# Cathoven-AI/Montreal-Forced-Aligner

Hardware: AMD Instinct MI355X
Metric: aligned utterances/sec (whole node), 10 s utts, 5k-state triphone (higher is better)
Workload: dtype f32 scores from 2-way f16-split products (3*2^-22 per term worst case), f64 path costs

## Files before the change

### include/mfa_hip.h

```cpp
#ifndef MFA_HIP_H_
#define MFA_HIP_H_

#include <stddef.h>
#include <stdint.h>

#ifdef __cplusplus
extern "C" {
#endif

#define MFA_API __attribute__((visibility("default")))

typedef struct mfa_ctx mfa_ctx;

MFA_API mfa_ctx *mfa_create(int device_id);
MFA_API void mfa_destroy(mfa_ctx *ctx);
MFA_API const char *mfa_last_error(mfa_ctx *ctx);
MFA_API int mfa_version(void);
MFA_API int mfa_set_stream(mfa_ctx *ctx, void *hip_stream, int use_own);
MFA_API int mfa_synchronize(mfa_ctx *ctx);
MFA_API void *mfa_device_alloc(mfa_ctx *ctx, size_t bytes);
MFA_API int mfa_device_free(mfa_ctx *ctx, void *d_ptr);
MFA_API int mfa_memcpy_h2d(mfa_ctx *ctx, void *d_dst, const void *h_src, size_t bytes);
MFA_API int mfa_memcpy_d2h(mfa_ctx *ctx, void *h_dst, const void *d_src, size_t bytes);
MFA_API int mfa_timer_begin(mfa_ctx *ctx);
MFA_API int mfa_timer_end_ms(mfa_ctx *ctx, float *h_ms);
MFA_API int mfa_kernel_timing(mfa_ctx *ctx, int enable);
MFA_API int mfa_kernel_time_ms(mfa_ctx *ctx, int which, float *h_ms, int *h_launches);
MFA_API int mfa_kernel_time_reset(mfa_ctx *ctx);

typedef struct {
  float sample_frequency;
  float frame_length_ms;
  float frame_shift_ms;
  float preemphasis;
  float low_frequency;
  float high_frequency;
  float cepstral_lifter;
  float energy_floor;
  int32_t num_mel_bins;
  int32_t num_coefficients;
  int32_t snip_edges;
  int32_t remove_dc_offset;
  int32_t use_energy;
  int32_t raw_energy;
} mfa_mfcc_opts;

MFA_API int mfa_mfcc_configure(mfa_ctx *ctx, const mfa_mfcc_opts *opts);
MFA_API int32_t mfa_mfcc_num_frames(mfa_ctx *ctx, int64_t num_samples);
MFA_API int mfa_mfcc_batch(mfa_ctx *ctx, const int16_t *d_pcm, const int64_t *d_sample_off, const int64_t *d_frame_off,
                           int32_t n_utt, int32_t max_frames, float *d_mfcc);

MFA_API int mfa_gather_pcm(int32_t n_utt, const int16_t *const *h_src, const int64_t *h_sample_off, int16_t *h_dst,
                           int32_t n_threads);

MFA_API int64_t mfa_resample_num_samples(int32_t in_hz, int32_t out_hz, int64_t n);
MFA_API int mfa_resample_plan(int32_t in_hz, int32_t out_hz, int32_t *phases, int32_t *in_per_unit, int32_t *max_taps,
                              int32_t *h_first, int32_t *h_taps, float *h_weights);
MFA_API int mfa_resample_plan_general(int32_t in_hz, int32_t out_hz, double cutoff_hz, int32_t zeros, int32_t *phases,
                                      int32_t *in_per_unit, int32_t *max_taps, int32_t *h_first, int32_t *h_taps,
                                      float *h_weights);
MFA_API int32_t mfa_resample_block_outputs(void);
MFA_API int mfa_resample_batch(mfa_ctx *ctx, int32_t in_hz, int32_t out_hz, const int16_t *d_in, const int64_t *d_in_off,
                               int16_t *d_out, const int64_t *d_out_off, const int32_t *d_utt, int32_t n_sel, int64_t max_out);

typedef struct {
  float sample_frequency;
  float frame_length_ms;
  float frame_shift_ms;
  float min_f0;
  float max_f0;
  float soft_min_f0;
  float penalty_factor;
  float lowpass_cutoff;
  float resample_frequency;
  float delta_pitch;
  float nccf_ballast;
  float preemphasis;
  float pov_scale;
  float pov_offset;
  float pitch_scale;
  int32_t lowpass_filter_width;
  int32_t upsample_filter_width;
  int32_t snip_edges;
// ... 208 lines not shown
```

### montreal_forced_aligner_amd/_lib.py

```python
from __future__ import annotations

import ctypes as C
import os
import subprocess
from pathlib import Path

_PKG = Path(__file__).resolve().parent
_SO = Path(os.environ["MFA_HIP_SO"]).resolve() if os.environ.get("MFA_HIP_SO") else _PKG / "libmfa_hip.so"
_SOURCES = ["api.hip", "mfcc.hip", "feats.hip", "gmm.hip", "gmm_band.hip", "gmm_pack.cpp", "score_plan.cpp", "viterbi.hip", "viterbi_general.hip",
            "fmllr.hip", "gmm_acc.hip", "gmm_acc_host.cpp", "resample.hip", "resample_plan.cpp", "pitch.hip", "pitch_plan.cpp", "compress.hip", "align_equal.hip", "align_equal_host.cpp",
            "lda_acc.hip", "lda_acc_host.cpp", "mllt_acc.hip", "mllt_acc_host.cpp", "tree_acc.hip", "tree_acc_host.cpp"]
_LIB = None


class MfaHipError(RuntimeError):
    pass


STATUS_REASONS = {
    2: "no alignment within the retry beam",
    3: "token capacity exceeded (device decoder status 3)",
    4: "back-pointer capacity exceeded (device decoder status 4)",
    5: "unsupported graph: a state with more than 64 arcs of a kind (device decoder status 5)",
    6: "internal consistency check failed (device decoder status 6)",
# ... 69 lines not shown
               "resample_plan.hpp", "pitch_plan.hpp", "compress_math.hpp", "gmm_acc_math.hpp", "tid_lookup.hpp", "align_equal_math.hpp", "lda_acc_math.hpp", "mllt_acc_math.hpp", "tree_acc_math.hpp")
    deps = srcs + [src_dir / h for h in headers] + [_PKG.parent / "include" / "mfa_hip.h"]
    if not force and _SO.exists() and all(_SO.stat().st_mtime >= d.stat().st_mtime for d in deps if d.exists()):
        return _SO
    hipcc = os.environ.get("HIPCC", "/opt/rocm/bin/hipcc")
    cmd = [hipcc, "--offload-arch=gfx950", "-O3", "-ffp-contract=off", "-fPIC", "-shared", "-std=c++17",
           "-fvisibility=hidden"] + os.environ.get("MFA_HIPCC_FLAGS", "").split() + ["-o", str(_SO)] + [str(s) for s in srcs]
    if verbose:
        print(" ".join(cmd))
    subprocess.check_call(cmd)
    return _SO


_vp, _i32, _i64, _f32 = C.c_void_p, C.c_int32, C.c_int64, C.c_float
SIGNATURES = {
    "mfa_create": (_vp, [C.c_int]),
    "mfa_destroy": (None, [_vp]),
    "mfa_last_error": (C.c_char_p, [_vp]),
    "mfa_version": (C.c_int, []),
    "mfa_set_stream": (C.c_int, [_vp, _vp, C.c_int]),
    "mfa_synchronize": (C.c_int, [_vp]),
    "mfa_device_alloc": (_vp, [_vp, C.c_size_t]),
    "mfa_device_free": (C.c_int, [_vp, _vp]),
    "mfa_memcpy_h2d": (C.c_int, [_vp, _vp, _vp, C.c_size_t]),
    "mfa_memcpy_d2h": (C.c_int, [_vp, _vp, _vp, C.c_size_t]),
    "mfa_timer_begin": (C.c_int, [_vp]),
    "mfa_timer_end_ms": (C.c_int, [_vp, C.POINTER(C.c_float)]),
    "mfa_kernel_timing": (C.c_int, [_vp, C.c_int]),
    "mfa_kernel_time_ms": (C.c_int, [_vp, C.c_int, C.POINTER(C.c_float), C.POINTER(C.c_int)]),
    "mfa_kernel_time_reset": (C.c_int, [_vp]),
    "mfa_mfcc_configure": (C.c_int, [_vp, C.POINTER(MfccOpts)]),
    "mfa_mfcc_num_frames": (_i32, [_vp, _i64]),
    "mfa_mfcc_batch": (C.c_int, [_vp, _vp, _vp, _vp, _i32, _i32, _vp]),
    "mfa_gather_pcm": (C.c_int, [_i32, _vp, _vp, _vp, _i32]),
    "mfa_resample_num_samples": (_i64, [_i32, _i32, _i64]),
    "mfa_resample_plan": (C.c_int, [_i32, _i32, _vp, _vp, _vp, _vp, _vp, _vp]),
    "mfa_resample_plan_general": (C.c_int, [_i32, _i32, C.c_double, _i32, _vp, _vp, _vp, _vp, _vp, _vp]),
    "mfa_resample_block_outputs": (_i32, []),
    "mfa_resample_batch": (C.c_int, [_vp, _i32, _i32, _vp, _vp, _vp, _vp, _vp, _i32, _i64]),
    "mfa_pitch_configure": (C.c_int, [_vp, C.POINTER(PitchOpts)]),
    "mfa_pitch_num_frames": (_i32, [_vp, _i64]),
    "mfa_pitch_num_states": (_i32, [_vp]),
    "mfa_pitch_num_columns": (_i32, [_vp]),
    "mfa_pitch_workspace_bytes": (C.c_size_t, [_vp, _i32, _i64, _i64, _i64, _i32]),
    "mfa_pitch_batch": (C.c_int, [_vp, _vp, _vp, _vp, _vp, _vp, _i32, _i32, _vp]),
    "mfa_pitch_process_batch": (C.c_int, [_vp, _vp, _vp, _i32, _i32, _vp, _i32, _i32]),
    "mfa_debug_pitch_stages": (C.c_int, [_vp, C.POINTER(PitchOpts), _vp, _vp, _vp, _vp, _vp, _vp, _vp, _vp, _vp, _vp, _vp, _vp,
                                         _i32, _i32, _vp, _vp, _vp, _vp, _vp, _vp]),
    "mfa_cmvn_stats": (C.c_int, [_vp, _vp, _vp, _i32, _i32, _vp, _vp, _i32, _vp]),
    "mfa_feats_batch": (C.c_int, [_vp, _vp, _vp, _i32, _i32, _i32, _vp, _vp, _i32, _i32, _vp, _i32, _i32, _vp, _vp]),
    "mfa_compress_resident_values": (_i32, []),
    "mfa_compress_batch": (C.c_int, [_vp, _vp, _vp, _i32, _i32, _i32, _i32, _vp, _vp, _i32, _vp, _vp, _vp, _vp]),
    "mfa_debug_compress_host": (C.c_int, [_vp, _i32, _i32, _vp, _vp, _vp, _vp]),
    "mfa_load_gmm": (C.c_int, [_vp, _i32, _i32, _vp, _vp, _vp, _vp]),
    "mfa_gmm_slot": (_i32, [_vp, _i32]),
    "mfa_gmm_sort_pdf_list": (C.c_int, [_vp, _vp, _i32, _vp]),
    "mfa_gmm_sort_pdf_list_keyed": (C.c_int, [_vp, _vp, _vp, _i32, _vp]),
    "mfa_fst_first_frames": (C.c_int, [_i32, _vp, _vp, _i32, _vp]),
    "mfa_debug_gmm_trace": (C.c_int, [_vp, _vp]),
    "mfa_debug_gmm_pack": (C.c_int, [_i32, _i32, _vp, _vp, _vp, _vp, _vp, _vp, _vp, _vp, _vp, _vp, _vp, _vp, _vp, _vp, _vp,
                                      _vp, _vp, _i32, _vp]),
    "mfa_debug_viterbi_stamps": (C.c_int, [_vp, _vp]),
    "mfa_gmm_score_batch": (C.c_int, [_vp, _vp, _vp, _i32, _i32, _vp, _vp, _vp, _vp, _vp, _vp]),
    "mfa_align_batch": (C.c_int, [_vp, C.POINTER(GraphBatch), _vp, _vp, _vp, _vp, _i64, _i64, _i32, _i32, C.POINTER(AlignOpts),
                                  _vp, _vp, _vp, _vp, _vp, _vp]),
    "mfa_align_general_batch": (C.c_int, [_vp, C.POINTER(GraphBatch), _vp, _vp, _vp, _vp, _vp, _i32, _i32, C.POINTER(AlignOpts),
# ... 6 lines not shown
    "mfa_build_score_plans_batch": (C.c_int, [_i32, _vp, _vp, _vp, _vp, _vp, _vp, _i32, _vp, _i32, _i32, _i32, _vp, _vp, _vp, _vp,
                                              _vp, _vp, _vp, _vp, _vp]),
    "mfa_fmllr_acc_batch": (C.c_int, [_vp, _vp, _vp, _i32, _i64, _vp, _vp, _vp, _vp, _i32, _vp, _vp, _vp]),
    "mfa_fmllr_acc_ali_batch": (C.c_int, [_vp, _vp, _vp, _i32, _i64, _vp, _vp, _vp, _i32, _vp, _vp, _vp, _vp, _i32, _vp, _vp, _vp]),
    "mfa_fmllr_stats_model": (C.c_int, [_vp, _i32, _i32, _vp, _vp, _vp]),
    "mfa_gmm_acc_chunk_frames": (_i32, []),
    "mfa_gmm_acc_max_dim": (_i32, []),
    "mfa_gmm_acc_batch": (C.c_int, [_vp, _vp, _i64, _vp, _vp, _vp, _i32, _vp, _vp, _vp, _vp, _vp]),
    "mfa_debug_gmm_acc_host": (C.c_int, [_i32, _i32, _vp, _vp, _vp, _vp, _vp, _i64, _vp, _vp, _vp, _i32, _vp, _vp, _vp, _vp, _vp,
                                          _vp, _i32]),
    "mfa_align_equal_batch": (C.c_int, [_vp, C.POINTER(GraphBatch), _vp, _i64, _i64, _vp, C.c_uint32, _vp, _vp]),
    "mfa_debug_align_equal_host": (C.c_int, [_i32, _vp, _vp, _vp, _vp, _vp, _vp, _vp, _vp, _vp, C.c_uint32, _vp, _vp]),
    "mfa_lda_acc_slab_frames": (_i32, []),
    "mfa_lda_acc_chunk_frames": (_i32, []),
    "mfa_lda_acc_max_dim": (_i32, []),
    "mfa_lda_acc_batch": (C.c_int, [_vp, _vp, _vp, _i32, _i64, _i32, _vp, _vp, _i32, _vp, _vp, _vp, _i32, _i32, _f32, _vp, C.c_uint32,
                                    _vp, _vp, _vp, _vp]),
    "mfa_debug_lda_acc_host": (C.c_int, [_vp, _vp, _i32, _i32, _vp, _vp, _i32, _vp, _vp, _vp, _i32, _i32, _f32, _vp, C.c_uint32,
                                         _vp, _vp, _vp, _vp]),
    "mfa_mllt_acc_chunk_frames": (_i32, []),
    "mfa_mllt_acc_max_dim": (_i32, []),
    "mfa_mllt_acc_batch": (C.c_int, [_vp, _vp, _i64, _vp, _vp, _vp, _i32, _vp, _vp, _vp, _vp]),
    "mfa_debug_mllt_acc_host": (C.c_int, [_i32, _i32, _vp, _vp, _vp, _vp, _vp, _vp, _i64, _vp, _vp, _vp, _vp, _vp, _vp, _i32]),
    "mfa_tree_acc_chunk_frames": (_i32, []),
    "mfa_tree_acc_max_dim": (_i32, []),
    "mfa_tree_acc_batch": (C.c_int, [_vp, _vp, _vp, _i32, _i64, _i32, _vp, _vp, _vp, _vp, _i32, _vp, _i32, _i64, _vp, _vp, _vp, _vp,
                                     _vp, _vp, _vp]),
    "mfa_debug_tree_acc_host": (C.c_int, [_vp, _vp, _i32, _i32, _vp, _vp, _vp, _vp, _i32, _vp, _i32, _i64, _vp, _vp, _vp, _vp, _vp,
                                          _vp, _vp]),
    "mfa_align_workspace_bytes": (C.c_size_t, [_vp, _i32, _i64, C.POINTER(AlignOpts)]),
}


def lib() -> C.CDLL:
    global _LIB
    if _LIB is None:
        if not _SO.exists():
            raise MfaHipError(
                f"{_SO} is missing: build it with `python -c 'import __graft_entry__ as g; g.build()'` "
                "(the alignment path has no CPU fallback)"
            )
        import torch

        try:
            handle = C.CDLL(str(_SO))
        except OSError as e:
            raise MfaHipError(f"cannot load {_SO}: {e}") from e
        for name, (res, args) in SIGNATURES.items():
            fn = getattr(handle, name)
            fn.restype = res
            fn.argtypes = args
        _LIB = handle
    return _LIB


def check(ctx, rc: int, what: str) -> None:
    if rc != 0:
        msg = lib().mfa_last_error(ctx)
        raise MfaHipError(f"{what}: {msg.decode() if msg else 'error'}")


def _ptr(t):
    return None if t is None else C.c_void_p(t.data_ptr())
```

### montreal_forced_aligner_amd/csrc/mfcc.hip

```cpp
#include <algorithm>
#include <cmath>
#include <vector>

#include "ctx.hpp"

namespace {

typedef float v2f __attribute__((ext_vector_type(2)));

constexpr int kNfft = 512;
constexpr int kHalf = 256;
#ifndef MFA_MFCC_WAVES
#define MFA_MFCC_WAVES 8
#endif
constexpr int kWavesPerBlock = MFA_MFCC_WAVES;
constexpr int kFramesPerWave = 16;
constexpr int kFramesPerBlock = kWavesPerBlock * kFramesPerWave;
constexpr int kMaxBins = 32;
constexpr int kMaxCeps = 16;
constexpr int kMaxDct = 384;
constexpr int kMaxPieces = 96;
constexpr int kPieceTaps = 8;
constexpr int kMaxMelW = kMaxPieces * kPieceTaps;
constexpr int kRowPad = 17;
constexpr int kTileFloats = 4 * 16 * kRowPad * 2;
constexpr int kPStride = 273;
constexpr int kPartStride = kMaxPieces + 8;
constexpr int kMelStride = kMaxBins + 8;
constexpr int kPartOff = 4 * kPStride;
constexpr int kMelOff = kPartOff + 4 * kPartStride;
static_assert(kMelOff + 4 * kMelStride <= kTileFloats, "tile reuse");

struct MfccParams {
  int win, shift, nbins, nceps, snip_edges, remove_dc;
  int n_pieces, n_rounds, np_max;
  int raw_energy;
  float log_energy_floor;
  float preemph;
  const float *window;
  const float *tw256;
  const float *tw512;
  const float *melw;
  const int32_t *melinfo;
  const float *dct;
  const float *lifter;
};

#define WAVE_SYNC()                                              \
  do {                                                           \
    __builtin_amdgcn_fence(__ATOMIC_RELEASE, "wavefront");       \
    __builtin_amdgcn_wave_barrier();                             \
    __builtin_amdgcn_fence(__ATOMIC_ACQUIRE, "wavefront");       \
  } while (0)

template <int CTRL>
__device__ __forceinline__ float dpp_f32(float old, float v) {
  return __int_as_float(__builtin_amdgcn_update_dpp(__float_as_int(old), __float_as_int(v), CTRL, 0xF, 0xF, false));
}
template <int CTRL>
__device__ __forceinline__ float dpp_perm(float v) {
  return __int_as_float(__builtin_amdgcn_mov_dpp(__float_as_int(v), CTRL, 0xF, 0xF, true));
}
__device__ __forceinline__ float row_sum_exact(float v) {
  v += dpp_f32<0xB1>(0.0f, v);
// ... 14 lines not shown
template <bool kZero3 = false>
__device__ __forceinline__ void dft4(v2f &a0, v2f &a1, v2f &a2, v2f &a3) {
  const v2f s02 = a0 + a2, d02 = a0 - a2;
  const v2f s13 = kZero3 ? a1 : a1 + a3, d13 = kZero3 ? a1 : a1 - a3;
  a0 = s02 + s13; a2 = s02 - s13;
  a1 = (v2f){d02.x + d13.y, d02.y - d13.x};
  a3 = (v2f){d02.x - d13.y, d02.y + d13.x};
}
template <int kLive = 16>
__device__ __forceinline__ void dft16(v2f (&a)[16]) {
  constexpr float c1 = 0.92387953251128674f, s1 = 0.38268343236508977f, h = 0.70710678118654752f;
#pragma unroll
  for (int na = 0; na < 4; na++) {
    if (na + 12 >= kLive && na + 8 < kLive) dft4<true>(a[na], a[na + 4], a[na + 8], a[na + 12]);
    else dft4<false>(a[na], a[na + 4], a[na + 8], a[na + 12]);
  }
  a[1 + 4] = cmul(a[1 + 4], (v2f){c1, -s1});
  a[1 + 8] = cmul(a[1 + 8], (v2f){h, -h});
  a[1 + 12] = cmul(a[1 + 12], (v2f){s1, -c1});
  a[2 + 4] = cmul(a[2 + 4], (v2f){h, -h});
  a[2 + 8] = (v2f){a[2 + 8].y, -a[2 + 8].x};
  a[2 + 12] = cmul(a[2 + 12], (v2f){-h, -h});
  a[3 + 4] = cmul(a[3 + 4], (v2f){s1, -c1});
  a[3 + 8] = cmul(a[3 + 8], (v2f){-h, -h});
  a[3 + 12] = cmul(a[3 + 12], (v2f){-c1, s1});
#pragma unroll
  for (int kb = 0; kb < 4; kb++) dft4(a[4 * kb], a[4 * kb + 1], a[4 * kb + 2], a[4 * kb + 3]);
#pragma unroll
  for (int kb = 0; kb < 4; kb++)
#pragma unroll
    for (int ka = kb + 1; ka < 4; ka++) { const v2f t = a[4 * kb + ka]; a[4 * kb + ka] = a[4 * ka + kb]; a[4 * ka + kb] = t; }
}

template <int kJ, bool kEnergy = false>
__global__ __launch_bounds__(64 * kWavesPerBlock, 4) void mfcc_kernel(MfccParams p, const int16_t *__restrict__ pcm,
                                                                        const int64_t *__restrict__ sample_off,
                                                                        const int64_t *__restrict__ frame_off,
                                                                        float *__restrict__ out) {
  __shared__ float s_tile[kWavesPerBlock][kTileFloats];
  __shared__ v2f s_tw256[256];
  __shared__ v2f s_tw512[256];
  __shared__ float s_melw[kMaxMelW];
  __shared__ float s_dct[kMaxDct];
  __shared__ v2f s_wnd[256];
  __shared__ int s_info[kMaxPieces + kMaxBins];
  const int utt = blockIdx.y;
  const int lane = threadIdx.x & 63, wave = __builtin_amdgcn_readfirstlane(threadIdx.x >> 6);
  const int q = lane >> 4, i = lane & 15;
  const int64_t s0 = sample_off[utt], n = sample_off[utt + 1] - s0;
  const int64_t f0 = frame_off[utt];
  const int T = (int)(frame_off[utt + 1] - f0);
  if ((int)blockIdx.x * kFramesPerBlock >= T) return;
  for (int k = threadIdx.x; k < 256; k += 64 * kWavesPerBlock) {
    s_tw256[k] = (v2f){p.tw256[2 * k], p.tw256[2 * k + 1]};
    s_tw512[k] = (v2f){p.tw512[2 * k], p.tw512[2 * k + 1]};
    s_wnd[k] = (v2f){p.window[2 * k], p.window[2 * k + 1]};
  }
  for (int k = threadIdx.x; k < p.n_pieces * kPieceTaps; k += 64 * kWavesPerBlock) s_melw[k] = p.melw[k];
  for (int k = threadIdx.x; k < p.nceps * p.nbins; k += 64 * kWavesPerBlock) s_dct[k] = p.dct[k];
  for (int k = threadIdx.x; k < kMaxPieces + kMaxBins; k += 64 * kWavesPerBlock) s_info[k] = p.melinfo[k];
  float *tile = s_tile[wave];
  for (int k = lane; k < kTileFloats; k += 64) tile[k] = 0.0f;
  __syncthreads();
  const int fbase = blockIdx.x * kFramesPerBlock + wave * kFramesPerWave;
  const int nfr = min(kFramesPerWave, T - fbase);
  if (nfr <= 0) return;
  const int16_t *x = pcm + s0;

  const float lift_k = i < p.nceps ? p.lifter[i] : 0.0f;
  v2f *tq = (v2f *)tile + q * (16 * kRowPad);
  float *pq = tile + q * kPStride;
  float *partq = tile + kPartOff + q * kPartStride;
  float *melq = tile + kMelOff + q * kMelStride;

  auto load_frame = [&](int f, unsigned (&raw)[kJ]) {
    const int64_t start = p.snip_edges ? (int64_t)f * p.shift : (int64_t)p.shift * f + p.shift / 2 - p.win / 2;
    const bool fast = start >= 0 && start + 32 * kJ <= n && (((s0 + start) & 1) == 0);
    if (__all(fast)) {
      const unsigned *xs = reinterpret_cast<const unsigned *>(x + start);
#pragma unroll
      for (int j = 0; j < kJ; j++) raw[j] = xs[16 * j + i];
      return;
    }
#pragma unroll
    for (int j = 0; j < kJ; j++) {
      unsigned both = 0;
#pragma unroll
      for (int e = 0; e < 2; e++) {
        const int s = 2 * (16 * j + i) + e;
        unsigned val = 0;
        if (s < p.win) {
          int64_t si = start + s;
          while (si < 0 || si >= n) si = (si < 0) ? (-si - 1) : (2 * n - 1 - si);
          val = (unsigned short)x[si];
        }
        both |= val << (16 * e);
      }
      raw[j] = both;
    }
  };
  auto frame_of = [&](int it) { return fbase + min(4 * it + q, nfr - 1); };

  unsigned nxt[kJ];
  load_frame(frame_of(0), nxt);
  const int npass = (nfr + 3) >> 2;
  for (int it = 0; it < npass; it++) {
    const int f = frame_of(it);
    const bool live = 4 * it + q < nfr;
    int ti = i;
    asm volatile("" : "+v"(ti));
    const v2f *wnd = s_wnd + ti, *tw256 = s_tw256 + ti, *tw512 = s_tw512 + ti;
    v2f a[16];
#pragma unroll
    for (int j = 0; j < 16; j++) a[j] = (v2f){0.0f, 0.0f};
#pragma unroll
    for (int j = 0; j < kJ; j++) a[j] = (v2f){(float)(short)(nxt[j] & 0xFFFFu), (float)(short)(nxt[j] >> 16)};
    if (it + 1 < npass) load_frame(frame_of(it + 1), nxt);
    const bool ok_e = 2 * (16 * (kJ - 1) + i) < p.win, ok_o = 2 * (16 * (kJ - 1) + i) + 1 < p.win;
    auto clear_tail = [&]() {
      if (p.win < 32 * (kJ - 1)) {
#pragma unroll
        for (int j = 8; j < kJ - 1; j++) {
          if (2 * (16 * j + i) >= p.win) a[j].x = 0.0f;
          if (2 * (16 * j + i) + 1 >= p.win) a[j].y = 0.0f;
        }
      }
      if (!ok_e) a[kJ - 1].x = 0.0f;
      if (!ok_o) a[kJ - 1].y = 0.0f;
    };
    clear_tail();
    float sum = 0.0f;
#pragma unroll
    for (int j = 0; j < kJ; j++) sum += a[j].x + a[j].y;
    sum = row_sum_exact(sum);
    const float off = p.remove_dc ? (-sum / (float)p.win) : 0.0f;
#pragma unroll
    for (int j = 0; j < kJ; j++) a[j] += splat(off);
    clear_tail();
    float log_energy = 0.0f;
    auto frame_log_energy = [&]() {
      float e = 0.0f;
#pragma unroll
      for (int j = 0; j < kJ; j++) e = fmaf(a[j].y, a[j].y, fmaf(a[j].x, a[j].x, e));
      e = row_sum_exact(e);
      return __builtin_amdgcn_logf(fmaxf(e, 1.1920928955078125e-07f)) * 0.693147180559945309f;
    };
    if constexpr (kEnergy) { if (p.raw_energy) log_energy = frame_log_energy(); }
    {
      float prev_e[kJ];
#pragma unroll
      for (int j = 0; j < kJ; j++) {
        const float up = a[j > 0 ? j - 1 : 0].y;
        const float carry = j == 0 ? a[0].x : dpp_perm<0x121>(up);
        prev_e[j] = dpp_f32<0x111>(carry, a[j].y);
      }
#pragma unroll
      for (int j = 0; j < kJ; j++) {
        const v2f prev = (v2f){prev_e[j], a[j].x};
        a[j] = (a[j] - splat(p.preemph) * prev) * wnd[16 * j];
      }
    }
    if constexpr (kEnergy) { if (!p.raw_energy) log_energy = frame_log_energy(); }
    dft16<kJ>(a);
#pragma unroll
    for (int k1 = 1; k1 < 16; k1++) a[k1] = cmul(a[k1], tw256[16 * k1]);
#pragma unroll
    for (int k1 = 0; k1 < 16; k1++) tq[k1 * kRowPad + i] = a[k1];
    WAVE_SYNC();
#pragma unroll
    for (int n2 = 0; n2 < 16; n2++) a[n2] = tq[i * kRowPad + n2];
    WAVE_SYNC();
    dft16(a);
#pragma unroll
    for (int k2 = 0; k2 < 16; k2++) {
      const v2f zk = a[k2], own = a[(16 - k2) & 15], far = a[15 - k2];
      const float cx = dpp_f32<0x111>(own.x, dpp_perm<0x140>(far.x));
      const float cy = dpp_f32<0x111>(own.y, dpp_perm<0x140>(far.y));
      float ex = zk.x + cx, ey = zk.y - cy, dx = zk.x - cx, dy = zk.y + cy;
      asm("" : "+v"(ex), "+v"(dx));
      const v2f xk = (v2f){ex, ey} + cmul(tw512[16 * k2], (v2f){dx, dy});
      float pw = 0.25f * fmaf(xk.y, xk.y, xk.x * xk.x);
      if (k2 == 0 && i == 0) pw = 0.25f * (xk.x * xk.x);
      pq[16 * k2 + i] = pw;
    }
    WAVE_SYNC();
    for (int r = 0; r < p.n_rounds; r++) {
      const int piece = 16 * r + i;
      const int pc = min(piece, p.n_pieces - 1);
      const float *wv = s_melw + pc * kPieceTaps;
      const float *pv = pq + s_info[pc];
      float acc = 0.0f;
#pragma unroll
      for (int t = 0; t < kPieceTaps; t++) acc = fmaf(wv[t], pv[t], acc);
      if (piece < p.n_pieces) partq[piece] = acc;
    }
    WAVE_SYNC();
#pragma unroll
    for (int half = 0; half < 2; half++) {
      const int b = i + 16 * half;
      if (b < p.nbins) {
        const int info = s_info[kMaxPieces + b];
        const int first = info & 0xFF, np = info >> 8;
        float e = partq[first];
        for (int r = 1; r < p.np_max; r++) if (r < np) e += partq[first + r];
        melq[b] = __builtin_amdgcn_logf(fmaxf(e, 1.1920928955078125e-07f)) * 0.693147180559945309f;
      }
    }
    WAVE_SYNC();
    if (i < p.nceps) {
      const float *d = s_dct + i * p.nbins;
      float acc = 0.0f;
      for (int b = 0; b < p.nbins; b++) acc = fmaf(d[b], melq[b], acc);
      float c_out = acc * lift_k;
      if constexpr (kEnergy) { if (i == 0) c_out = fmaxf(log_energy, p.log_energy_floor); }
      if (live) out[(f0 + f) * p.nceps + i] = c_out;
    }
    WAVE_SYNC();
  }
}

float mel_scale(float f) { return 1127.0f * logf(1.0f + f / 700.0f); }

}

extern "C" {

MFA_API int mfa_mfcc_configure(mfa_ctx *c, const mfa_mfcc_opts *o) {
  MFA_HIP_CHECK(c, hipSetDevice(c->device));
  int win = (int)(o->sample_frequency * 0.001f * o->frame_length_ms);
  int shift = (int)(o->sample_frequency * 0.001f * o->frame_shift_ms);
  int nfft = 1;
  while (nfft < win) nfft <<= 1;
  if (nfft != kNfft) return c->fail("MFCC kernel supports a 512-point FFT (window %d samples → %d)", win, nfft);
  if (o->num_mel_bins > kMaxBins || o->num_coefficients > kMaxCeps || o->num_coefficients > o->num_mel_bins ||
      o->num_mel_bins * o->num_coefficients > kMaxDct)
    return c->fail("unsupported num_mel_bins/num_coefficients %d/%d", o->num_mel_bins, o->num_coefficients);
  int nb = o->num_mel_bins, nc = o->num_coefficients;
  std::vector<float> window(win);
  double a = 2.0 * M_PI / (win - 1);
  for (int i = 0; i < win; i++) window[i] = (float)pow(0.5 - 0.5 * cos(a * (double)i), 0.85);
  std::vector<float> wpairs(16 * 16 * 2, 0.0f);
  for (int j = 0; j < 16; j++)
    for (int i = 0; i < 16; i++)
      for (int e = 0; e < 2; e++) {
        const int sidx = 2 * (16 * j + i) + e;
        wpairs[2 * (16 * j + i) + e] = sidx < win ? window[sidx] : 0.0f;
      }
  std::vector<float> tw(2 * 256 * 2);
  for (int k = 0; k < 16; k++)
    for (int i = 0; i < 16; i++) {
      const double a256 = 2.0 * M_PI * (double)(i * k) / 256.0, a512 = 2.0 * M_PI * (double)(i + 16 * k) / 512.0;
      tw[2 * (16 * k + i)] = (float)cos(a256);
      tw[2 * (16 * k + i) + 1] = (float)(-sin(a256));
      tw[512 + 2 * (16 * k + i)] = (float)(-sin(a512));
// ... 44 lines not shown
      for (int t = 0; t < best_taps; t++) {
        const int at = q * best_taps + t;
        piecew.push_back(at < len_of[b] ? melw[woff_of[b] + at] : 0.0f);
      }
    }
  }
  std::vector<float> dct((size_t)nc * nb), lifter(nc);
  float norm0 = std::sqrt(1.0f / (float)nb), norm = std::sqrt(2.0f / (float)nb);
  for (int k = 0; k < nc; k++)
    for (int n = 0; n < nb; n++)
      dct[(size_t)k * nb + n] = (k == 0) ? norm0 : (float)(norm * std::cos((double)M_PI / nb * (n + 0.5) * k));
  for (int i = 0; i < nc; i++)
    lifter[i] = o->cepstral_lifter != 0.0f ? (float)(1.0 + 0.5 * o->cepstral_lifter * sin(M_PI * i / o->cepstral_lifter)) : 1.0f;

  return dev_upload_commit<MfaHipDev>(
      c, "the MFCC tables",
      {{&c->d_window, wpairs.data(), wpairs.size() * 4}, {&c->d_twiddle, tw.data(), tw.size() * 4},
       {&c->d_melw, piecew.data(), piecew.size() * 4}, {&c->d_melidx, melinfo.data(), melinfo.size() * 4},
       {&c->d_dct, dct.data(), dct.size() * 4}, {&c->d_lifter, lifter.data(), lifter.size() * 4}},
      [&] {
        c->n_melw = n_pieces; c->mel_np_max = np_max;
        c->mfcc = *o;
        c->win = win; c->shift = shift; c->nfft = nfft;
        c->mfcc_ready = true;
      });
}

MFA_API int32_t mfa_mfcc_num_frames(mfa_ctx *c, int64_t n) {
  if (!c->mfcc_ready) return -1;
  if (c->mfcc.snip_edges) return n < c->win ? 0 : (int32_t)(1 + (n - c->win) / c->shift);
  return (int32_t)((n + c->shift / 2) / c->shift);
}

MFA_API int mfa_mfcc_batch(mfa_ctx *c, const int16_t *d_pcm, const int64_t *d_sample_off, const int64_t *d_frame_off,
                           int32_t n_utt, int32_t max_frames, float *d_mfcc) {
  if (!c->mfcc_ready) return c->fail("mfa_mfcc_configure has not been called");
  if (n_utt <= 0 || max_frames <= 0) return 0;
  if (n_utt > 65535) return c->fail("at most 65535 utterances per MFCC launch (got %d)", n_utt);
  MfccParams p;
  p.win = c->win; p.shift = c->shift; p.nbins = c->mfcc.num_mel_bins; p.nceps = c->mfcc.num_coefficients;
  p.snip_edges = c->mfcc.snip_edges; p.remove_dc = c->mfcc.remove_dc_offset; p.preemph = c->mfcc.preemphasis;
  p.raw_energy = c->mfcc.raw_energy;
  p.log_energy_floor = c->mfcc.energy_floor > 0.0f ? logf(c->mfcc.energy_floor) : -INFINITY;
  p.window = c->d_window.ptr<float>(); p.tw256 = c->d_twiddle.ptr<float>(); p.tw512 = p.tw256 + 512;
  p.melw = c->d_melw.ptr<float>(); p.melinfo = c->d_melidx.ptr<int32_t>(); p.dct = c->d_dct.ptr<float>(); p.lifter = c->d_lifter.ptr<float>();
  p.n_pieces = c->n_melw; p.n_rounds = (c->n_melw + 15) / 16; p.np_max = c->mel_np_max;
  dim3 grid((max_frames + kFramesPerBlock - 1) / kFramesPerBlock, n_utt);
  KernelTimer kt(c, MFA_K_MFCC);
  const bool energy = c->mfcc.use_energy != 0;
  if (c->win <= 32 * 13) {
    if (energy) hipLaunchKernelGGL((mfcc_kernel<13, true>), grid, dim3(64 * kWavesPerBlock), 0, c->stream, p, d_pcm, d_sample_off, d_frame_off, d_mfcc);
    else hipLaunchKernelGGL((mfcc_kernel<13, false>), grid, dim3(64 * kWavesPerBlock), 0, c->stream, p, d_pcm, d_sample_off, d_frame_off, d_mfcc);
  } else {
    if (energy) hipLaunchKernelGGL((mfcc_kernel<16, true>), grid, dim3(64 * kWavesPerBlock), 0, c->stream, p, d_pcm, d_sample_off, d_frame_off, d_mfcc);
    else hipLaunchKernelGGL((mfcc_kernel<16, false>), grid, dim3(64 * kWavesPerBlock), 0, c->stream, p, d_pcm, d_sample_off, d_frame_off, d_mfcc);
  }
  MFA_HIP_CHECK(c, hipGetLastError());
  return 0;
}

}
```

### montreal_forced_aligner_amd/engine.py

```python
from __future__ import annotations

import ctypes as C
from functools import partialmethod
from typing import Dict, List, Optional, Sequence

import numpy as np
import torch

from . import _lib, hostcpu
from ._lib import AlignOpts, GraphBatch, MfccOpts, ScorePlan, _ptr, check
from .frontend import DEFAULT_PITCH, _PITCH_ALIAS, FrontEndStages
from .kaldi_io import Fst
from .model import DiagGmmModel, TransitionModel
from .packing import GraphPacking, PackedGraphs
from .pipeline import Pipeline
from .ragged import _rows_by_group, _speaker_groups, max_len, offsets
from .staging import StagingPool, StagingRing
from .stats import (GmmStats, LdaStats, MlltStats, TreeStats, check_delta_fmllr, fmllr_statistics, gmm_statistics, gmm_statistics_host,
                    lda_statistics, lda_statistics_host, mllt_statistics, mllt_statistics_host, model_arrays, tid_tables, tree_statistics, tree_statistics_host)

STATUS_OK, STATUS_RETRIED, STATUS_FAILED, STATUS_TOKEN_OVERFLOW, STATUS_BP_OVERFLOW, STATUS_UNSUPPORTED = 0, 1, 2, 3, 4, 5

DEFAULT_MFCC = dict(sample_frequency=16000.0, frame_length_ms=25.0, frame_shift_ms=10.0, preemphasis=0.97,
                    low_frequency=20.0, high_frequency=7800.0, cepstral_lifter=22.0, energy_floor=0.0,
# ... 24 lines not shown
        self.use_torch_stream()
        self.mfcc_opts: Optional[MfccOpts] = None
        self.num_ceps = 13
        self.gmm: Optional[DiagGmmModel] = None
        self.slot_class: Optional[np.ndarray] = None
        self._staging = StagingRing(self.device, 3)
        self._pcm_staging = StagingRing(self.device, 2)
        self._nf_checked: Optional[tuple] = None
        self._slab, self._slab_off = None, 0

    def next_staging(self) -> StagingPool:
        return self._staging.next()

    def close(self) -> None:
        if self.ctx:
            self.lib.mfa_destroy(self.ctx)
            self.ctx = None

    def __del__(self):
        try:
            self.close()
        except Exception:
            pass

    def use_torch_stream(self) -> None:
        self.stream = torch.cuda.current_stream(self.device)
        check(self.ctx, self.lib.mfa_set_stream(self.ctx, C.c_void_p(self.stream.cuda_stream), 0), "mfa_set_stream")

    def configure_mfcc(self, **kw) -> None:
        opts = _lib.options(MfccOpts, DEFAULT_MFCC, kw, "MFCC")
        check(self.ctx, self.lib.mfa_mfcc_configure(self.ctx, C.byref(opts)), "mfa_mfcc_configure")
        self.mfcc_opts = opts
        self.num_ceps = int(opts.num_coefficients)

    def load_gmm(self, gmm: DiagGmmModel) -> None:
        po, gc, mi, iv = model_arrays(gmm)
        check(self.ctx, self.lib.mfa_load_gmm(self.ctx, gmm.dim, gmm.num_pdfs, po.ctypes.data, gc.ctypes.data,
                                              mi.ctypes.data, iv.ctypes.data), "mfa_load_gmm")
        self.gmm = gmm
        slots = np.array([self.lib.mfa_gmm_slot(self.ctx, p) for p in range(gmm.num_pdfs)], dtype=np.int32)
        n_gauss = np.diff(gmm.pdf_offsets)
        cls = np.full(gmm.num_pdfs, 5, dtype=np.int32)
        for i, s in enumerate((32, 16, 8, 4, 1)):
            cls[slots == s] = i + 1
        cls[(slots == 32) & (n_gauss <= 32)] = 0
        self.slot_class = cls

    def num_frames(self, num_samples: int) -> int:
        return int(self.lib.mfa_mfcc_num_frames(self.ctx, num_samples))

    def num_frames_array(self, num_samples: np.ndarray) -> np.ndarray:
        n = np.asarray(num_samples, dtype=np.int64)
        if self.mfcc_opts is None:
            self.configure_mfcc()
        o = self.mfcc_opts
        f32 = np.float32
        win = int(f32(f32(o.sample_frequency) * f32(0.001)) * f32(o.frame_length_ms))
        shift = int(f32(f32(o.sample_frequency) * f32(0.001)) * f32(o.frame_shift_ms))
        snip = int(o.snip_edges)
        out = np.where(n < win, 0, 1 + (n - win) // shift) if snip else (n + shift // 2) // shift
        key = (win, shift, snip)
        if self._nf_checked != key:
            for probe in (0, 1, win - 1, win, win + shift - 1, win + shift, 159999, 160000, 160001, 1 << 20):
                ref = (0 if probe < win else 1 + (probe - win) // shift) if snip else (probe + shift // 2) // shift
                if self.num_frames(probe) != ref:
                    raise _lib.MfaHipError("num_frames_array disagrees with mfa_mfcc_num_frames")
# ... 252 lines not shown
```

Before: 264,100.

## Add specialised MFCC kernel path with lane-strided constant tables and fixed mel loops

Adds a specialised MFCC kernel variant that is picked when every mel bin spans at most 8 pieces. It re-lays the twiddle, window, mel-weight and DCT tables in shared memory with a per-lane stride so each lane can read them as 16-byte vectors. The mel-piece and bin loops become fixed-count unrolled loops with per-lane offsets held in registers. The aim is to cut LDS traffic, bank conflicts and loop overhead in the front end, at the cost of higher register pressure and more template instantiations. MFCC is a small share of the whole alignment pipeline, so end-to-end gains are likely small.

```diff
diff --git a/include/mfa_hip.h b/include/mfa_hip.h
--- a/include/mfa_hip.h
+++ b/include/mfa_hip.h
@@ -49,6 +49,7 @@
 MFA_API int32_t mfa_mfcc_num_frames(mfa_ctx *ctx, int64_t num_samples);
 MFA_API int mfa_mfcc_batch(mfa_ctx *ctx, const int16_t *d_pcm, const int64_t *d_sample_off, const int64_t *d_frame_off,
                            int32_t n_utt, int32_t max_frames, float *d_mfcc);
+MFA_API int mfa_mfcc_path(mfa_ctx *ctx);
 
 MFA_API int mfa_gather_pcm(int32_t n_utt, const int16_t *const *h_src, const int64_t *h_sample_off, int16_t *h_dst,
                            int32_t n_threads);
diff --git a/montreal_forced_aligner_amd/_lib.py b/montreal_forced_aligner_amd/_lib.py
--- a/montreal_forced_aligner_amd/_lib.py
+++ b/montreal_forced_aligner_amd/_lib.py
@@ -125,6 +125,7 @@
     "mfa_mfcc_configure": (C.c_int, [_vp, C.POINTER(MfccOpts)]),
     "mfa_mfcc_num_frames": (_i32, [_vp, _i64]),
     "mfa_mfcc_batch": (C.c_int, [_vp, _vp, _vp, _vp, _i32, _i32, _vp]),
+    "mfa_mfcc_path": (C.c_int, [_vp]),
     "mfa_gather_pcm": (C.c_int, [_i32, _vp, _vp, _vp, _i32]),
     "mfa_resample_num_samples": (_i64, [_i32, _i32, _i64]),
     "mfa_resample_plan": (C.c_int, [_i32, _i32, _vp, _vp, _vp, _vp, _vp, _vp]),
@@ -197,6 +198,9 @@
 }
 
 
+_NEWER = {"mfa_mfcc_path"}
+
+
 def lib() -> C.CDLL:
     global _LIB
     if _LIB is None:
@@ -212,6 +216,8 @@
         except OSError as e:
             raise MfaHipError(f"cannot load {_SO}: {e}") from e
         for name, (res, args) in SIGNATURES.items():
+            if name in _NEWER and os.environ.get("MFA_HIP_SO") and not hasattr(handle, name):
+                continue
             fn = getattr(handle, name)
             fn.restype = res
             fn.argtypes = args
diff --git a/montreal_forced_aligner_amd/csrc/mfcc.hip b/montreal_forced_aligner_amd/csrc/mfcc.hip
--- a/montreal_forced_aligner_amd/csrc/mfcc.hip
+++ b/montreal_forced_aligner_amd/csrc/mfcc.hip
@@ -7,6 +7,7 @@
 namespace {
 
 typedef float v2f __attribute__((ext_vector_type(2)));
+typedef float v4f __attribute__((ext_vector_type(4)));
 
 constexpr int kNfft = 512;
 constexpr int kHalf = 256;
@@ -30,6 +31,17 @@
 constexpr int kPartOff = 4 * kPStride;
 constexpr int kMelOff = kPartOff + 4 * kPartStride;
 static_assert(kMelOff + 4 * kMelStride <= kTileFloats, "tile reuse");
+constexpr int kFastRounds = kMaxPieces / 16;
+constexpr int kFastNp = 8;
+static_assert(kMaxPieces + kFastNp <= kPartStride + 1, "a bin's batch of piece sums stays inside its row");
+static_assert(kMelOff % 4 == 0 && kMelStride % 4 == 0 && kTileFloats % 4 == 0, "16-byte reads of the log energies");
+constexpr int kLaneStride = 36;
+constexpr int kGenTw256 = 0, kGenTw512 = 512, kGenWnd = 1024, kGenMelw = 1536, kGenDct = kGenMelw + kMaxMelW,
+              kGenInfo = kGenDct + kMaxDct, kGenConst = kGenInfo + kMaxPieces + kMaxBins;
+constexpr int kFastTab = 16 * kLaneStride;
+constexpr int kFastTw256 = 0, kFastTw512 = kFastTab, kFastWnd = 2 * kFastTab, kFastMelw = 3 * kFastTab,
+              kFastDct = kFastMelw + kMaxMelW, kFastConst = kFastDct + kMaxCeps * kLaneStride;
+static_assert(kMaxBins <= kLaneStride - 4 && kFastMelw % 4 == 0 && kFastDct % 4 == 0, "16-byte units");
 
 struct MfccParams {
   int win, shift, nbins, nceps, snip_edges, remove_dc;
@@ -110,18 +122,15 @@
     for (int ka = kb + 1; ka < 4; ka++) { const v2f t = a[4 * kb + ka]; a[4 * kb + ka] = a[4 * ka + kb]; a[4 * ka + kb] = t; }
 }
 
-template <int kJ, bool kEnergy = false>
+template <int kJ, bool kEnergy, bool kFast>
 __global__ __launch_bounds__(64 * kWavesPerBlock, 4) void mfcc_kernel(MfccParams p, const int16_t *__restrict__ pcm,
                                                                         const int64_t *__restrict__ sample_off,
                                                                         const int64_t *__restrict__ frame_off,
                                                                         float *__restrict__ out) {
-  __shared__ float s_tile[kWavesPerBlock][kTileFloats];
-  __shared__ v2f s_tw256[256];
-  __shared__ v2f s_tw512[256];
-  __shared__ float s_melw[kMaxMelW];
-  __shared__ float s_dct[kMaxDct];
-  __shared__ v2f s_wnd[256];
-  __shared__ int s_info[kMaxPieces + kMaxBins];
+  __shared__ __attribute__((aligned(16))) float s_tile[kWavesPerBlock][kTileFloats];
+  __shared__ __attribute__((aligned(16))) float s_const[kFast ? kFastConst : kGenConst];
+  constexpr int kTw256 = kFast ? kFastTw256 : kGenTw256, kTw512 = kFast ? kFastTw512 : kGenTw512,
+                kWnd = kFast ? kFastWnd : kGenWnd, kMelw = kFast ? kFastMelw : kGenMelw, kDct = kFast ? kFastDct : kGenDct;
   const int utt = blockIdx.y;
   const int lane = threadIdx.x & 63, wave = __builtin_amdgcn_readfirstlane(threadIdx.x >> 6);
   const int q = lane >> 4, i = lane & 15;
@@ -130,13 +139,25 @@
   const int T = (int)(frame_off[utt + 1] - f0);
   if ((int)blockIdx.x * kFramesPerBlock >= T) return;
   for (int k = threadIdx.x; k < 256; k += 64 * kWavesPerBlock) {
-    s_tw256[k] = (v2f){p.tw256[2 * k], p.tw256[2 * k + 1]};
-    s_tw512[k] = (v2f){p.tw512[2 * k], p.tw512[2 * k + 1]};
-    s_wnd[k] = (v2f){p.window[2 * k], p.window[2 * k + 1]};
-  }
-  for (int k = threadIdx.x; k < p.n_pieces * kPieceTaps; k += 64 * kWavesPerBlock) s_melw[k] = p.melw[k];
-  for (int k = threadIdx.x; k < p.nceps * p.nbins; k += 64 * kWavesPerBlock) s_dct[k] = p.dct[k];
-  for (int k = threadIdx.x; k < kMaxPieces + kMaxBins; k += 64 * kWavesPerBlock) s_info[k] = p.melinfo[k];
+    const int at = kFast ? (k & 15) * kLaneStride + 2 * (k >> 4) : 2 * k;
+    s_const[kTw256 + at] = p.tw256[2 * k]; s_const[kTw256 + at + 1] = p.tw256[2 * k + 1];
+    s_const[kTw512 + at] = p.tw512[2 * k]; s_const[kTw512 + at + 1] = p.tw512[2 * k + 1];
+    s_const[kWnd + at] = p.window[2 * k]; s_const[kWnd + at + 1] = p.window[2 * k + 1];
+  }
+  if constexpr (kFast) {
+    for (int k = threadIdx.x; k < kMaxMelW; k += 64 * kWavesPerBlock) {
+      const int piece = k / kPieceTaps, t = k % kPieceTaps;
+      s_const[kMelw + (((piece >> 4) * 2 + (t >> 2)) * 16 + (piece & 15)) * 4 + (t & 3)] = piece < p.n_pieces ? p.melw[k] : 0.0f;
+    }
+    for (int k = threadIdx.x; k < kMaxCeps * kLaneStride; k += 64 * kWavesPerBlock) {
+      const int row = k / kLaneStride, b = k % kLaneStride;
+      s_const[kDct + k] = row < p.nceps && b < p.nbins ? p.dct[row * p.nbins + b] : 0.0f;
+    }
+  } else {
+    for (int k = threadIdx.x; k < p.n_pieces * kPieceTaps; k += 64 * kWavesPerBlock) s_const[kMelw + k] = p.melw[k];
+    for (int k = threadIdx.x; k < p.nceps * p.nbins; k += 64 * kWavesPerBlock) s_const[kDct + k] = p.dct[k];
+    for (int k = threadIdx.x; k < kMaxPieces + kMaxBins; k += 64 * kWavesPerBlock) s_const[kGenInfo + k] = __int_as_float(p.melinfo[k]);
+  }
   float *tile = s_tile[wave];
   for (int k = lane; k < kTileFloats; k += 64) tile[k] = 0.0f;
   __syncthreads();
@@ -145,22 +166,34 @@
   if (nfr <= 0) return;
   const int16_t *x = pcm + s0;
 
-  const float lift_k = i < p.nceps ? p.lifter[i] : 0.0f;
+  auto lane_lifter = [&](int l) { return l < p.nceps ? p.lifter[l] : 0.0f; };
   v2f *tq = (v2f *)tile + q * (16 * kRowPad);
   float *pq = tile + q * kPStride;
   float *partq = tile + kPartOff + q * kPartStride;
   float *melq = tile + kMelOff + q * kMelStride;
-
-  auto load_frame = [&](int f, unsigned (&raw)[kJ]) {
+  auto lane_plan = [&](int l, int (&poff)[kFastRounds], int (&binfo)[2]) {
+#pragma unroll
+    for (int r = 0; r < kFastRounds; r++) poff[r] = p.melinfo[16 * r + l];
+    binfo[0] = p.melinfo[kMaxPieces + l]; binfo[1] = p.melinfo[kMaxPieces + 16 + l];
+  };
+  constexpr bool kKeep = kJ <= 13;
+  float lift_k = 0.0f;
+  int poff[kFastRounds] = {}, binfo[2] = {};
+  if constexpr (kKeep) {
+    lift_k = lane_lifter(i);
+    if constexpr (kFast) lane_plan(i, poff, binfo);
+  }
+
+  auto load_frame = [&](int f, int li, unsigned (&raw)[kJ]) {
     const int64_t start = p.snip_edges ? (int64_t)f * p.shift : (int64_t)p.shift * f + p.shift / 2 - p.win / 2;
     const bool fast = start >= 0 && start + 32 * kJ <= n && (((s0 + start) & 1) == 0);
     if (__all(fast)) {
       const unsigned *xs = reinterpret_cast<const unsigned *>(x + start);
 #pragma unroll
-      for (int j = 0; j < kJ; j++) raw[j] = xs[16 * j + i];
+      for (int j = 0; j < kJ; j++) raw[j] = xs[16 * j + li];
       return;
     }
-#pragma unroll
+#pragma unroll 1
     for (int j = 0; j < kJ; j++) {
       unsigned both = 0;
 #pragma unroll
@@ -174,26 +207,45 @@
         }
         both |= val << (16 * e);
       }
-      raw[j] = both;
+#pragma unroll
+      for (int jj = 0; jj < kJ; jj++) raw[jj] = jj == j ? both : raw[jj];
     }
   };
   auto frame_of = [&](int it) { return fbase + min(4 * it + q, nfr - 1); };
+  auto load_tab = [&](const float *tab, int at, int first, int kN, v2f (&w)[16]) {
+    if constexpr (kFast) {
+#pragma unroll
+      for (int c = 0; c < 8; c++)
+        if (2 * c < kN) {
+          v4f t = *reinterpret_cast<const v4f *>(tab + at + 4 * c);
+          asm("" : "+v"(t));
+          w[2 * c] = (v2f){t.x, t.y}; w[2 * c + 1] = (v2f){t.z, t.w};
+        }
+    } else {
+#pragma unroll
+      for (int e = 0; e < 16; e++)
+        if (e >= first && e < kN) w[e] = *reinterpret_cast<const v2f *>(tab + at + 32 * e);
+    }
+  };
 
   unsigned nxt[kJ];
-  load_frame(frame_of(0), nxt);
+#pragma unroll
+  for (int j = 0; j < kJ; j++) nxt[j] = 0;
+  load_frame(frame_of(0), i, nxt);
   const int npass = (nfr + 3) >> 2;
   for (int it = 0; it < npass; it++) {
     const int f = frame_of(it);
     const bool live = 4 * it + q < nfr;
     int ti = i;
     asm volatile("" : "+v"(ti));
-    const v2f *wnd = s_wnd + ti, *tw256 = s_tw256 + ti, *tw512 = s_tw512 + ti;
+    const int tab_at = kFast ? ti * kLaneStride : 2 * ti;
+    const int li = kKeep ? i : ti;
     v2f a[16];
 #pragma unroll
     for (int j = 0; j < 16; j++) a[j] = (v2f){0.0f, 0.0f};
 #pragma unroll
     for (int j = 0; j < kJ; j++) a[j] = (v2f){(float)(short)(nxt[j] & 0xFFFFu), (float)(short)(nxt[j] >> 16)};
-    if (it + 1 < npass) load_frame(frame_of(it + 1), nxt);
+    if (it + 1 < npass) load_frame(frame_of(it + 1), li, nxt);
     const bool ok_e = 2 * (16 * (kJ - 1) + i) < p.win, ok_o = 2 * (16 * (kJ - 1) + i) + 1 < p.win;
     auto clear_tail = [&]() {
       if (p.win < 32 * (kJ - 1)) {
@@ -225,6 +277,8 @@
     };
     if constexpr (kEnergy) { if (p.raw_energy) log_energy = frame_log_energy(); }
     {
+      v2f w[16];
+      load_tab(s_const + kWnd, tab_at, 0, kJ, w);
       float prev_e[kJ];
 #pragma unroll
       for (int j = 0; j < kJ; j++) {
@@ -235,69 +289,128 @@
 #pragma unroll
       for (int j = 0; j < kJ; j++) {
         const v2f prev = (v2f){prev_e[j], a[j].x};
-        a[j] = (a[j] - splat(p.preemph) * prev) * wnd[16 * j];
+        a[j] = (a[j] - splat(p.preemph) * prev) * w[j];
       }
     }
     if constexpr (kEnergy) { if (!p.raw_energy) log_energy = frame_log_energy(); }
     dft16<kJ>(a);
-#pragma unroll
-    for (int k1 = 1; k1 < 16; k1++) a[k1] = cmul(a[k1], tw256[16 * k1]);
-#pragma unroll
-    for (int k1 = 0; k1 < 16; k1++) tq[k1 * kRowPad + i] = a[k1];
+    {
+      v2f w[16];
+      load_tab(s_const + kTw256, tab_at, 1, 16, w);
+#pragma unroll
+      for (int k1 = 1; k1 < 16; k1++) a[k1] = cmul(a[k1], w[k1]);
+    }
+#pragma unroll
+    for (int k1 = 0; k1 < 16; k1++) tq[k1 * kRowPad + li] = a[k1];
     WAVE_SYNC();
 #pragma unroll
-    for (int n2 = 0; n2 < 16; n2++) a[n2] = tq[i * kRowPad + n2];
+    for (int n2 = 0; n2 < 16; n2++) a[n2] = tq[li * kRowPad + n2];
     WAVE_SYNC();
     dft16(a);
-#pragma unroll
-    for (int k2 = 0; k2 < 16; k2++) {
-      const v2f zk = a[k2], own = a[(16 - k2) & 15], far = a[15 - k2];
-      const float cx = dpp_f32<0x111>(own.x, dpp_perm<0x140>(far.x));
-      const float cy = dpp_f32<0x111>(own.y, dpp_perm<0x140>(far.y));
-      float ex = zk.x + cx, ey = zk.y - cy, dx = zk.x - cx, dy = zk.y + cy;
-      asm("" : "+v"(ex), "+v"(dx));
-      const v2f xk = (v2f){ex, ey} + cmul(tw512[16 * k2], (v2f){dx, dy});
-      float pw = 0.25f * fmaf(xk.y, xk.y, xk.x * xk.x);
-      if (k2 == 0 && i == 0) pw = 0.25f * (xk.x * xk.x);
-      pq[16 * k2 + i] = pw;
+    {
+      v2f w[16];
+      load_tab(s_const + kTw512, tab_at, 0, 16, w);
+#pragma unroll
+      for (int k2 = 0; k2 < 16; k2++) {
+        const v2f zk = a[k2], own = a[(16 - k2) & 15], far = a[15 - k2];
+        const float cx = dpp_f32<0x111>(own.x, dpp_perm<0x140>(far.x));
+        const float cy = dpp_f32<0x111>(own.y, dpp_perm<0x140>(far.y));
+        float ex = zk.x + cx, ey = zk.y - cy, dx = zk.x - cx, dy = zk.y + cy;
+        asm("" : "+v"(ex), "+v"(dx));
+        const v2f xk = (v2f){ex, ey} + cmul(w[k2], (v2f){dx, dy});
+        float pw = 0.25f * fmaf(xk.y, xk.y, xk.x * xk.x);
+        if (k2 == 0 && i == 0) pw = 0.25f * (xk.x * xk.x);
+        pq[16 * k2 + li] = pw;
+      }
     }
     WAVE_SYNC();
-    for (int r = 0; r < p.n_rounds; r++) {
-      const int piece = 16 * r + i;
-      const int pc = min(piece, p.n_pieces - 1);
-      const float *wv = s_melw + pc * kPieceTaps;
-      const float *pv = pq + s_info[pc];
+    float c_out;
+    if constexpr (kFast) {
+      if constexpr (!kKeep) lane_plan(ti, poff, binfo);
+      const float *mw = s_const + kMelw + 4 * ti;
+      float psum[kFastRounds];
+#pragma unroll
+      for (int r = 0; r < kFastRounds; r++) {
+        const v4f wa = *reinterpret_cast<const v4f *>(mw + (2 * r) * 64), wb = *reinterpret_cast<const v4f *>(mw + (2 * r + 1) * 64);
+        const float *pv = pq + poff[r];
+        float acc = 0.0f;
+        acc = fmaf(wa.x, pv[0], acc); acc = fmaf(wa.y, pv[1], acc); acc = fmaf(wa.z, pv[2], acc); acc = fmaf(wa.w, pv[3], acc);
+        acc = fmaf(wb.x, pv[4], acc); acc = fmaf(wb.y, pv[5], acc); acc = fmaf(wb.z, pv[6], acc); acc = fmaf(wb.w, pv[7], acc);
+        psum[r] = acc;
+      }
+#pragma unroll
+      for (int r = 0; r < kFastRounds; r++) partq[16 * r + li] = psum[r];
+      WAVE_SYNC();
+      float v[2][kFastNp];
+#pragma unroll
+      for (int half = 0; half < 2; half++)
+#pragma unroll
+        for (int r = 0; r < kFastNp; r++) v[half][r] = partq[(binfo[half] & 0xFF) + r];
+#pragma unroll
+      for (int half = 0; half < 2; half++) {
+        const int np = binfo[half] >> 8;
+        float e = v[half][0];
+#pragma unroll
+        for (int r = 1; r < kFastNp; r++) e += r < np ? v[half][r] : 0.0f;
+        const float le = __builtin_amdgcn_logf(fmaxf(e, 1.1920928955078125e-07f)) * 0.693147180559945309f;
+        v[half][0] = np > 0 ? le : 0.0f;
+      }
+      melq[li] = v[0][0]; melq[li + 16] = v[1][0];
+      WAVE_SYNC();
+      const float *d = s_const + kDct + tab_at;
       float acc = 0.0f;
 #pragma unroll
-      for (int t = 0; t < kPieceTaps; t++) acc = fmaf(wv[t], pv[t], acc);
-      if (piece < p.n_pieces) partq[piece] = acc;
-    }
+      for (int c = 0; c < kMaxBins / 4; c++) {
+        const v4f dw = *reinterpret_cast<const v4f *>(d + 4 * c), m = *reinterpret_cast<const v4f *>(melq + 4 * c);
+        acc = fmaf(dw.x, m.x, acc); acc = fmaf(dw.y, m.y, acc); acc = fmaf(dw.z, m.z, acc); acc = fmaf(dw.w, m.w, acc);
+      }
+      c_out = acc * (kKeep ? lift_k : lane_lifter(ti));
+    } else {
+      const float *s_melw = s_const + kMelw, *s_dct = s_const + kDct, *s_info = s_const + kGenInfo;
+      for (int r = 0; r < p.n_rounds; r++) {
+        const int piece = 16 * r + i;
+        const int pc = min(piece, p.n_pieces - 1);
+        const float *wv = s_melw + pc * kPieceTaps;
+        const float *pv = pq + __float_as_int(s_info[pc]);
+        float acc = 0.0f;
+#pragma unroll
+        for (int t = 0; t < kPieceTaps; t++) acc = fmaf(wv[t], pv[t], acc);
+        if (piece < p.n_pieces) partq[piece] = acc;
+      }
+      WAVE_SYNC();
+#pragma unroll
+      for (int half = 0; half < 2; half++) {
+        const int b = i + 16 * half;
+        if (b < p.nbins) {
+          const int info = __float_as_int(s_info[kMaxPieces + b]);
+          const int first = info & 0xFF, np = info >> 8;
+          float e = partq[first];
+          for (int r = 1; r < p.np_max; r++) if (r < np) e += partq[first + r];
+          melq[b] = __builtin_amdgcn_logf(fmaxf(e, 1.1920928955078125e-07f)) * 0.693147180559945309f;
+        }
+      }
+      WAVE_SYNC();
+      float acc = 0.0f;
+      if (i < p.nceps) {
+        const float *d = s_dct + i * p.nbins;
+        for (int b = 0; b < p.nbins; b++) acc = fmaf(d[b], melq[b], acc);
+      }
+      c_out = acc * (kKeep ? lift_k : lane_lifter(ti));
+    }
+    if constexpr (kEnergy) { if (i == 0) c_out = fmaxf(log_energy, p.log_energy_floor); }
+    if (i < p.nceps && live) out[(f0 + f) * p.nceps + li] = c_out;
     WAVE_SYNC();
-#pragma unroll
-    for (int half = 0; half < 2; half++) {
-      const int b = i + 16 * half;
-      if (b < p.nbins) {
-        const int info = s_info[kMaxPieces + b];
-        const int first = info & 0xFF, np = info >> 8;
-        float e = partq[first];
-        for (int r = 1; r < p.np_max; r++) if (r < np) e += partq[first + r];
-        melq[b] = __builtin_amdgcn_logf(fmaxf(e, 1.1920928955078125e-07f)) * 0.693147180559945309f;
-      }
-    }
-    WAVE_SYNC();
-    if (i < p.nceps) {
-      const float *d = s_dct + i * p.nbins;
-      float acc = 0.0f;
-      for (int b = 0; b < p.nbins; b++) acc = fmaf(d[b], melq[b], acc);
-      float c_out = acc * lift_k;
-      if constexpr (kEnergy) { if (i == 0) c_out = fmaxf(log_energy, p.log_energy_floor); }
-      if (live) out[(f0 + f) * p.nceps + i] = c_out;
-    }
-    WAVE_SYNC();
   }
 }
 
 float mel_scale(float f) { return 1127.0f * logf(1.0f + f / 700.0f); }
+
+template <int kJ, bool kEnergy, bool kFast>
+void mfcc_launch(mfa_ctx *c, dim3 grid, const MfccParams &p, const int16_t *d_pcm, const int64_t *d_sample_off,
+                        const int64_t *d_frame_off, float *d_mfcc) {
+  hipLaunchKernelGGL((mfcc_kernel<kJ, kEnergy, kFast>), grid, dim3(64 * kWavesPerBlock), 0, c->stream, p, d_pcm, d_sample_off,
+                     d_frame_off, d_mfcc);
+}
 
 }
 
@@ -408,6 +521,13 @@
   return (int32_t)((n + c->shift / 2) / c->shift);
 }
 
+MFA_API int mfa_mfcc_path(mfa_ctx *c) {
+  if (!c->mfcc_ready) return 0;
+  const char *generic = getenv("MFA_MFCC_GENERIC");
+  const bool force_generic = generic && generic[0] == '1';
+  return !force_generic && c->mel_np_max <= kFastNp ? 1 : 2;
+}
+
 MFA_API int mfa_mfcc_batch(mfa_ctx *c, const int16_t *d_pcm, const int64_t *d_sample_off, const int64_t *d_frame_off,
                            int32_t n_utt, int32_t max_frames, float *d_mfcc) {
   if (!c->mfcc_ready) return c->fail("mfa_mfcc_configure has not been called");
@@ -423,13 +543,16 @@
   p.n_pieces = c->n_melw; p.n_rounds = (c->n_melw + 15) / 16; p.np_max = c->mel_np_max;
   dim3 grid((max_frames + kFramesPerBlock - 1) / kFramesPerBlock, n_utt);
   KernelTimer kt(c, MFA_K_MFCC);
-  const bool energy = c->mfcc.use_energy != 0;
-  if (c->win <= 32 * 13) {
-    if (energy) hipLaunchKernelGGL((mfcc_kernel<13, true>), grid, dim3(64 * kWavesPerBlock), 0, c->stream, p, d_pcm, d_sample_off, d_frame_off, d_mfcc);
-    else hipLaunchKernelGGL((mfcc_kernel<13, false>), grid, dim3(64 * kWavesPerBlock), 0, c->stream, p, d_pcm, d_sample_off, d_frame_off, d_mfcc);
-  } else {
-    if (energy) hipLaunchKernelGGL((mfcc_kernel<16, true>), grid, dim3(64 * kWavesPerBlock), 0, c->stream, p, d_pcm, d_sample_off, d_frame_off, d_mfcc);
-    else hipLaunchKernelGGL((mfcc_kernel<16, false>), grid, dim3(64 * kWavesPerBlock), 0, c->stream, p, d_pcm, d_sample_off, d_frame_off, d_mfcc);
+  const int which = (c->win <= 32 * 13 ? 0 : 4) + (c->mfcc.use_energy != 0 ? 2 : 0) + (mfa_mfcc_path(c) == 1 ? 1 : 0);
+  switch (which) {
+    case 0: mfcc_launch<13, false, false>(c, grid, p, d_pcm, d_sample_off, d_frame_off, d_mfcc); break;
+    case 1: mfcc_launch<13, false, true>(c, grid, p, d_pcm, d_sample_off, d_frame_off, d_mfcc); break;
+    case 2: mfcc_launch<13, true, false>(c, grid, p, d_pcm, d_sample_off, d_frame_off, d_mfcc); break;
+    case 3: mfcc_launch<13, true, true>(c, grid, p, d_pcm, d_sample_off, d_frame_off, d_mfcc); break;
+    case 4: mfcc_launch<16, false, false>(c, grid, p, d_pcm, d_sample_off, d_frame_off, d_mfcc); break;
+    case 5: mfcc_launch<16, false, true>(c, grid, p, d_pcm, d_sample_off, d_frame_off, d_mfcc); break;
+    case 6: mfcc_launch<16, true, false>(c, grid, p, d_pcm, d_sample_off, d_frame_off, d_mfcc); break;
+    default: mfcc_launch<16, true, true>(c, grid, p, d_pcm, d_sample_off, d_frame_off, d_mfcc); break;
   }
   MFA_HIP_CHECK(c, hipGetLastError());
   return 0;
diff --git a/montreal_forced_aligner_amd/engine.py b/montreal_forced_aligner_amd/engine.py
--- a/montreal_forced_aligner_amd/engine.py
+++ b/montreal_forced_aligner_amd/engine.py
@@ -80,6 +80,9 @@
         check(self.ctx, self.lib.mfa_mfcc_configure(self.ctx, C.byref(opts)), "mfa_mfcc_configure")
         self.mfcc_opts = opts
         self.num_ceps = int(opts.num_coefficients)
+
+    def mfcc_path(self) -> str:
+        return {1: "specialised", 2: "generic"}[int(self.lib.mfa_mfcc_path(self.ctx))]
 
     def load_gmm(self, gmm: DiagGmmModel) -> None:
         po, gc, mi, iv = model_arrays(gmm)
```

Result: faster. 271,200, median of 6 (+2.7%).
